# snimu/mixture-of-tokenizers

Hardware: AMD Instinct MI355X
Metric: mixed-embed tokens/sec at BxT=256x2048; achieved HBM GB/s vs peak (higher is better)
Workload: dtype f32

## Files before the change

### mixture-of-tokenizers_amd/csrc/mot_embed.hip

```cpp
#include <stdlib.h>

#include <algorithm>

#include "mot_wave.hpp"

namespace mot {

template <int MODE, int NCH, int U, typename T, bool DUAL>
struct MixStream {
    typedef typename Elem<T>::vec vec_t;
    typedef typename Elem<T>::raw raw_t;
    static constexpr int VEC = Elem<T>::kVec;
    const MixArgs &A;
    const WaveLds &W;
    const T *tok_table, *byte_table;
    int lane, Dm, nchunk, ntok;
    int tokv = 0, unit_lane0 = 0;
    bool act[NCH];
    bool tact[NCH];
    raw_t ar[U][NCH];

    __device__ __forceinline__ MixStream(const MixArgs &A_, const WaveLds &W_, int ntok_) : A(A_), W(W_), ntok(ntok_) {
        tok_table = (const T *)A.tok_table;
        byte_table = (const T *)A.byte_table;
        lane = threadIdx.x & 63;
        Dm = MODE == MOT_MIX_CONCAT ? A.Dt + A.bpt * A.Db : A.Dt;
        nchunk = Dm / VEC;
#pragma unroll
        for (int i = 0; i < NCH; ++i) act[i] = lane + 64 * i < nchunk;
        if (MODE == MOT_MIX_CONCAT) {
#pragma unroll
            for (int i = 0; i < NCH; ++i) tact[i] = VEC * (lane + 64 * i) < A.Dt;
        }
    }
    __device__ __forceinline__ void request(int tb) {
#pragma unroll
        for (int u = 0; u < U; ++u) {
            const int t = min(tb + u, ntok - 1);
            int tok = __builtin_amdgcn_readlane(tokv, unit_lane0 + t);
            if ((uint64_t)(uint32_t)tok >= (uint64_t)A.tok_rows) {
                if (A.status && lane == 0) atomicOr(A.status, kStatusTokenOor);
                tok = 0;
            }
            if (MODE == MOT_MIX_CONCAT) {
                const T *trow = tok_table + (int64_t)tok * A.Dt;
#pragma unroll
                for (int i = 0; i < NCH; ++i) ar[u][i] = Elem<T>::load_raw(trow + VEC * (tact[i] ? lane + 64 * i : 0));
                continue;
            }
            const T *trow = tok_table + (int64_t)tok * Dm;
#pragma unroll
            for (int i = 0; i < NCH; ++i) ar[u][i] = Elem<T>::load_raw(trow + VEC * (act[i] ? lane + 64 * i : 0));
        }
    }
    template <class RowOf>
    __device__ __forceinline__ void run(RowOf &&out_row) {
        constexpr bool dual = DUAL;
        const int sv = A.bpt | 1;
        int slot[NCH], within[NCH];
#pragma unroll
        for (int i = 0; i < NCH; ++i) {
            const int c = lane + 64 * i;
            const int cc = act[i] ? c : 0;
            if (MODE == MOT_MIX_SUM) {
                slot[i] = (VEC * cc) / A.Db;
                within[i] = VEC * cc - slot[i] * A.Db;
            } else if (MODE == MOT_MIX_CONCAT) {
                const int cb = (act[i] && !tact[i]) ? VEC * c - A.Dt : 0;
                slot[i] = cb / A.Db;
                within[i] = cb - slot[i] * A.Db;
            } else {
                slot[i] = 0;
                within[i] = VEC * cc;
            }
        }
        const float s_tok = A.scale_tok ? *A.scale_tok : 1.0f;
        const float s_byte = A.scale_byte ? *A.scale_byte : 1.0f;
        const bool scale_t = A.scale_tok != nullptr, scale_b = A.scale_byte != nullptr;
        auto sumsq = [](const vec_t &v) {
            float s = 0.f;
#pragma unroll
            for (int e = 0; e < VEC; ++e) s += v[e] * v[e];
            return s;
        };

        for (int tb = 0; tb < ntok; tb += U) {
            raw_t br[U][NCH], br2[DUAL ? U : 1][NCH];
            vec_t bm[U][NCH];
            int idr[U][NCH];
            if (tb > 0) request(tb);
#pragma unroll
            for (int u = 0; u < U; ++u) {
                const int t = min(tb + u, ntok - 1);
#pragma unroll
                for (int i = 0; i < NCH; ++i) {
                    if (MODE == MOT_MIX_SUM || MODE == MOT_MIX_CONCAT) {
                        const int id = W.ids[t * sv + slot[i]];
                        idr[u][i] = id;
                        br[u][i] = Elem<T>::load_raw(byte_table + (int64_t)id * A.Db + within[i]);
                        if (dual) br2[DUAL ? u : 0][i] = Elem<T>::load_raw(byte_table + (int64_t)W.ids2[t * sv + slot[i]] * A.Db + within[i]);
                    } else if (MODE == MOT_MIX_MEAN) {
                        vec_t acc = (vec_t)(0.f);
                        for (int k = 0; k < A.bpt; ++k) {
                            const int id = W.ids[t * sv + k];
                            vec_t v = Elem<T>::loadv(byte_table + (int64_t)id * A.Db + within[i]);
                            if (dual) {
                                const int id2 = W.ids2[t * sv + k];
                                v += Elem<T>::loadv(byte_table + (int64_t)id2 * A.Db + within[i]);
                            }
                            if (A.norm_byte) v *= A.byte_rnorm[id];
                            acc += v;
                        }
                        bm[u][i] = acc / (float)A.bpt;
                    }
                }
            }
#pragma unroll
            for (int u = 0; u < U; ++u) {
                const int t = tb + u;
                vec_t a[1][NCH], b[1][NCH];
#pragma unroll
                for (int i = 0; i < NCH; ++i) {
                    a[0][i] = Elem<T>::widen(ar[u][i]);
                    if (MODE == MOT_MIX_SUM) {
                        vec_t v = Elem<T>::widen(br[u][i]);
                        if (dual) v += Elem<T>::widen(br2[DUAL ? u : 0][i]);
                        if (A.norm_byte) v *= A.byte_rnorm[idr[u][i]];
                        b[0][i] = v;
                    } else if (MODE == MOT_MIX_CONCAT) {
                        vec_t v = Elem<T>::widen(br[u][i]);
                        if (dual) v += Elem<T>::widen(br2[DUAL ? u : 0][i]);
                        if (A.norm_byte) {
                            if (dual) {
                                float ss = sumsq(v);
                                for (int o = 1; o < A.Db / VEC; o <<= 1) ss += __shfl_xor(ss, o, 64);
                                v *= rms_scale(ss, A.Db, A.eps);
                            } else {
                                v *= A.byte_rnorm[idr[u][i]];
                            }
                        }
                        b[0][i] = v;
                    } else if (MODE == MOT_MIX_MEAN) {
                        b[0][i] = bm[u][i];
                    }
                }
                if (A.norm_tok) {
                    float ss = 0.f;
#pragma unroll
                    for (int i = 0; i < NCH; ++i) ss += (MODE == MOT_MIX_CONCAT ? tact[i] : act[i]) ? sumsq(a[0][i]) : 0.f;
                    const float r = rms_scale(wave_sum(ss), MODE == MOT_MIX_CONCAT ? A.Dt : Dm, A.eps);
#pragma unroll
                    for (int i = 0; i < NCH; ++i) a[0][i] *= r;
                }
                if (scale_t) {
#pragma unroll
                    for (int i = 0; i < NCH; ++i) a[0][i] *= s_tok;
                }
                vec_t x[NCH];
#pragma unroll
                for (int i = 0; i < NCH; ++i) {
                    if (MODE == MOT_MIX_NOOP) x[i] = a[0][i];
                    else if (MODE == MOT_MIX_CONCAT) x[i] = tact[i] ? a[0][i] : (scale_b ? b[0][i] * s_byte : b[0][i]);
                    else x[i] = a[0][i] + (scale_b ? b[0][i] * s_byte : b[0][i]);
                }
                if (A.norm_out) {
                    float ss = 0.f;
#pragma unroll
                    for (int i = 0; i < NCH; ++i) ss += act[i] ? sumsq(x[i]) : 0.f;
                    const float r = rms_scale(wave_sum(ss), Dm, A.eps);
#pragma unroll
                    for (int i = 0; i < NCH; ++i) x[i] *= r;
                }
                if (t < ntok) {
                    T *orow = out_row(t);
#pragma unroll
                    for (int i = 0; i < NCH; ++i)
                        if (act[i]) Elem<T>::storev_nt(orow + VEC * (lane + 64 * i), x[i]);
                }
            }
        }
    }
};

template <int MODE, int NCH, int U, typename T, bool DUAL>
__global__ __launch_bounds__(kThreads) void embed_mix_kernel(const MixArgs A) {
    extern __shared__ __attribute__((aligned(16))) unsigned char lds_wave[];
    constexpr bool has_ids = MODE != MOT_MIX_NOOP;
    constexpr bool dual = DUAL;
    const int lane = threadIdx.x & 63;
    const int wave = __builtin_amdgcn_readfirstlane(threadIdx.x >> 6);
    const int64_t unit_id = (int64_t)blockIdx.x * kWaves + wave;
    if (unit_id >= A.n_units) return;
    const int64_t row = unit_id / A.units_per_row;
    const int64_t u0 = (unit_id - row * A.units_per_row) * A.unit;
    const int ntok = (int)min((int64_t)A.unit, A.T - u0);
    const int stream_eb = (has_ids && A.id_source == MOT_IDS_FROM_TTB && A.pull_dir != kPullNone) ? A.ttb_elem : 0;
    const WaveLds W = wave_lds_carve(lds_wave + (size_t)wave * A.wave_lds, A.unit, has_ids ? A.bpt : 0, dual, stream_eb);
    MixStream<MODE, NCH, U, T, DUAL> S(A, W, ntok);

    auto from_ttb = [&](auto indexer) {
        S.tokv = indexer.tokens();
        S.unit_lane0 = indexer.unit_lane0;
        indexer.load_rows();
#ifndef MOT_VAR_NOPREFETCH
        S.request(0);
#endif
        indexer.finish();
#ifdef MOT_VAR_NOPREFETCH
        S.request(0);
#endif
    };
    if (has_ids && A.id_source == MOT_IDS_FROM_TTB) {
        if (A.ttb_elem == 2) {
            if (A.pull_dir == kPullLeft) from_ttb(WaveIndexer<kPullLeft, int16_t>(A, W, row, u0, ntok, dual));
            else if (A.pull_dir == kPullRight) from_ttb(WaveIndexer<kPullRight, int16_t>(A, W, row, u0, ntok, dual));
            else from_ttb(WaveIndexer<kPullNone, int16_t>(A, W, row, u0, ntok, dual));
        } else {
            if (A.pull_dir == kPullLeft) from_ttb(WaveIndexer<kPullLeft, int32_t>(A, W, row, u0, ntok, dual));
            else if (A.pull_dir == kPullRight) from_ttb(WaveIndexer<kPullRight, int32_t>(A, W, row, u0, ntok, dual));
            else from_ttb(WaveIndexer<kPullNone, int32_t>(A, W, row, u0, ntok, dual));
        }
    } else {
        S.tokv = lane < ntok ? A.tokens[row * A.T + u0 + lane] : 0;
        S.request(0);
        if (has_ids) wave_ids_given(A, W, row, u0, ntok);
        else if (A.counters && lane == 0) atomicAdd((unsigned long long *)A.counters, (unsigned long long)ntok);
    }

    T *orow = (T *)A.out + (row * A.T + u0) * (int64_t)S.Dm;
    S.run([&](int t) { return orow + (int64_t)t * S.Dm; });
}

constexpr int kRouteUnits = 8;
constexpr int64_t kRouteMinTokens = 131072;
constexpr int kClaimShards = 64;
constexpr int kClaimStride = 64;

struct RouteWs {
    uint32_t *claim;
    uint8_t *ends;
    uint8_t *offs;
    uint16_t *ids;
    uint16_t *ids2;
};

template <int DIR, typename E>
__global__ __launch_bounds__(kThreads) void route_index_kernel(const MixArgs A, const RouteWs R) {
    extern __shared__ __attribute__((aligned(16))) unsigned char lds_wave[];
    const int lane = threadIdx.x & 63;
    const int wave = __builtin_amdgcn_readfirstlane(threadIdx.x >> 6);
    if (blockIdx.x < 2) R.claim[(blockIdx.x * kThreads + threadIdx.x) * kClaimStride] = 0;
    const int64_t unit_id = (int64_t)blockIdx.x * kWaves + wave;
    if (unit_id >= A.n_units) return;
    const int64_t row = unit_id / A.units_per_row;
    const int64_t u0 = (unit_id - row * A.units_per_row) * A.unit;
    const int ntok = (int)min((int64_t)A.unit, A.T - u0);
    const bool dual = A.add_padded != 0;
    const WaveLds W = wave_lds_carve(lds_wave + (size_t)wave * A.wave_lds, A.unit, A.bpt, dual, DIR != kPullNone ? A.ttb_elem : 0);
    WaveIndexer<DIR, E> ix(A, W, row, u0, ntok, dual);
    const int tok = ix.tokens();
    ix.load_rows();
    ix.finish();

    const int bpt = A.bpt, sv = bpt | 1, n = ntok * bpt;
    const int64_t base = (row * A.T + u0) * bpt;
    for (int i = lane; i < n; i += 64) {
        const int t = i / bpt, k = i - t * bpt;
        R.ids[base + i] = (uint16_t)W.ids[t * sv + k];
        if (dual) R.ids2[base + i] = (uint16_t)W.ids2[t * sv + k];
    }
    const bool in = ix.in_unit;
    const int b = tok & 7;
    int rank = 0, end = 0, acc = 0;
#pragma unroll
    for (int q = 0; q < 8; ++q) {
        const unsigned long long m = __ballot(in && b == q);
        if (in && b == q) rank = acc + (int)__builtin_amdgcn_mbcnt_hi((unsigned)(m >> 32), __builtin_amdgcn_mbcnt_lo((unsigned)m, 0u));
        acc += __popcll(m);
        if (lane == q) end = acc;
    }
    if (in) R.offs[unit_id * A.unit + rank] = (uint8_t)ix.j;
    if (lane < 8) R.ends[unit_id * 8 + lane] = (uint8_t)end;
}

template <int NCH, int U, typename T, bool DUAL>
__global__ __launch_bounds__(kThreads) void embed_mix_routed_kernel(const MixArgs A, const RouteWs R) {
    extern __shared__ __attribute__((aligned(16))) unsigned char lds_wave[];
    const int lane = threadIdx.x & 63;
    const int wave = __builtin_amdgcn_readfirstlane(threadIdx.x >> 6);
    const WaveLds W = wave_lds_carve(lds_wave + (size_t)wave * A.wave_lds, 64, A.bpt, DUAL, 0);
    MixStream<MOT_MIX_SUM, NCH, U, T, DUAL> S(A, W, 0);
    const int bpt = A.bpt, sv = bpt | 1;
    const int64_t n_chunks = (A.n_units + kRouteUnits - 1) / kRouteUnits;
    const int home = blockIdx.x & 7;
    const int shard = ((blockIdx.x >> 3) * kWaves + wave) % kClaimShards;
    for (int q = 0; q < 8;) {
        const int b = (home + q) & 7;
        const int64_t lo = n_chunks * shard / kClaimShards, hi = n_chunks * (shard + 1) / kClaimShards;
        uint32_t k = 0;
        if (lane == 0) k = atomicAdd(R.claim + (b * kClaimShards + shard) * kClaimStride, 1u);
        const int64_t c = lo + __builtin_amdgcn_readfirstlane(k);
        if (c >= hi) { ++q; continue; }
        const int64_t uc = c * kRouteUnits;
        int nb = 0, sb = 0;
        if (lane < kRouteUnits && uc + lane < A.n_units) {
            const uint8_t *e = R.ends + (uc + lane) * 8;
            sb = b ? e[b - 1] : 0;
            nb = e[b] - sb;
        }
        const int incl = wave_scan_add(nb), excl = incl - nb;
        const int total = __builtin_amdgcn_readlane(incl, kRouteUnits - 1);
        for (int p0 = 0; p0 < total; p0 += 64) {
            const int l = p0 + lane;
            int g = 0;
#pragma unroll
            for (int gg = 1; gg < kRouteUnits; ++gg) g = l >= __builtin_amdgcn_readlane(excl, gg) ? gg : g;
            const int ex = __shfl(excl, g, 64), st = __shfl(sb, g, 64);
            int64_t pos = 0;
            int tok = 0;
            if (l < total) {
                const int64_t u = uc + g;
                const int64_t row = u / A.units_per_row;
                pos = row * A.T + (u - row * A.units_per_row) * A.unit + R.offs[u * A.unit + st + (l - ex)];
                tok = A.tokens[pos];
                if ((uint64_t)(uint32_t)tok >= (uint64_t)A.ttb_rows) tok = 0;
            }
            S.tokv = tok;
            S.ntok = min(64, total - p0);
            S.request(0);
            if (l < total) {
                const uint16_t *ia = R.ids + pos * bpt, *ib = R.ids2 + pos * bpt;
                if ((bpt & 7) == 0) {
                    typedef uint16_t u16x8 __attribute__((ext_vector_type(8)));
                    for (int k = 0; k < bpt; k += 8) {
                        const u16x8 va = *(const u16x8 *)(ia + k);
                        u16x8 vb;
                        if (DUAL) vb = *(const u16x8 *)(ib + k);
#pragma unroll
                        for (int e = 0; e < 8; ++e) {
                            W.ids[lane * sv + k + e] = va[e];
                            if (DUAL) W.ids2[lane * sv + k + e] = vb[e];
                        }
                    }
                } else {
                    for (int k = 0; k < bpt; ++k) {
                        W.ids[lane * sv + k] = ia[k];
                        if (DUAL) W.ids2[lane * sv + k] = ib[k];
                    }
                }
            }
            wave_lds_sync();
            const int plo = (int)(uint32_t)pos, phi = (int)(pos >> 32);
            S.run([&](int t) {
                const int64_t p = (int64_t)(((uint64_t)(uint32_t)__builtin_amdgcn_readlane(phi, t) << 32) |
                                            (uint32_t)__builtin_amdgcn_readlane(plo, t));
                return (T *)A.out + p * (int64_t)S.Dm;
            });
            wave_lds_sync();
        }
    }
}

template <typename T>
__global__ __launch_bounds__(kThreads) void rows_rnorm_kernel(const T *__restrict__ table, int64_t rows, int dim,
                                                              float eps, float *__restrict__ out) {
    const int lane = threadIdx.x & 63;
    const int64_t r = (int64_t)blockIdx.x * kWaves + (threadIdx.x >> 6);
    if (r >= rows) return;
    float ss = 0.f;
    for (int j = lane; j < dim; j += 64) {
        const float v = Elem<T>::load1(table + r * dim + j);
        ss += v * v;
    }
    ss = wave_sum(ss);
    if (lane == 0) out[r] = rms_scale(ss, dim, eps);
}

template <int G, typename IdT, typename T>
__global__ __launch_bounds__(kThreads) void gather_rows_kernel(const IdT *__restrict__ ids_a, const IdT *__restrict__ ids_b,
                                                               int64_t n, const T *__restrict__ table, int64_t rows,
                                                               int dim, int rms, float eps, const float *scale,
                                                               T *__restrict__ out, uint32_t *status, int group, int64_t out_ld,
                                                               uint32_t oor_flag) {
    const int g = threadIdx.x % G;
    const int64_t per_block = kThreads / G;
    const float s = scale ? *scale : 1.0f;
    const bool vec = (dim & 3) == 0;
    for (int64_t r = (int64_t)blockIdx.x * per_block + threadIdx.x / G; r < n; r += (int64_t)gridDim.x * per_block) {
        int64_t ia = (int64_t)ids_a[r], ib = ids_b ? (int64_t)ids_b[r] : 0;
        if ((uint64_t)ia >= (uint64_t)rows || (uint64_t)ib >= (uint64_t)rows) {
            if (status) atomicOr(status, oor_flag);
            if ((uint64_t)ia >= (uint64_t)rows) ia = 0;
            if ((uint64_t)ib >= (uint64_t)rows) ib = 0;
        }
        const T *pa = table + ia * dim, *pb = table + ib * dim;
        T *po = group == 1 ? out + r * out_ld : out + (r / group) * out_ld + (r % group) * dim;
        float mult = s;
        if (rms) {
            float ss = 0.f;
            if (vec) {
                for (int j = g; j < (dim >> 2); j += G) {
                    float4v v = Elem<T>::load4(pa + 4 * j);
                    if (ids_b) v += Elem<T>::load4(pb + 4 * j);
                    ss += v.x * v.x + v.y * v.y + v.z * v.z + v.w * v.w;
                }
            } else {
                for (int j = g; j < dim; j += G) {
                    float v = Elem<T>::load1(pa + j);
                    if (ids_b) v += Elem<T>::load1(pb + j);
                    ss += v * v;
                }
            }
#pragma unroll
            for (int o = G / 2; o > 0; o >>= 1) ss += __shfl_xor(ss, o, G);
            mult = rms_scale(ss, dim, eps);
        }
        if (vec) {
            for (int j = g; j < (dim >> 2); j += G) {
                float4v v = Elem<T>::load4(pa + 4 * j);
                if (ids_b) v += Elem<T>::load4(pb + 4 * j);
                if (rms) v *= mult;
                if (scale) v *= s;
                Elem<T>::store4_nt(po + 4 * j, v);
            }
        } else {
            for (int j = g; j < dim; j += G) {
                float v = Elem<T>::load1(pa + j);
                if (ids_b) v += Elem<T>::load1(pb + j);
                if (rms) v *= mult;
                if (scale) v *= s;
                Elem<T>::store1(po + j, v);
            }
        }
    }
}

template <int G, typename T>
static int launch_gather_g(const void *ids_a, const void *ids_b, int ids_elem, int64_t n, const void *table,
                           int64_t rows, int dim, int rms, float eps, const float *scale, void *out, uint32_t *status,
                           int group, int64_t out_ld, uint32_t oor_flag, hipStream_t stream) {
    const int64_t per_block = kThreads / G;
    int64_t blocks = (n + per_block - 1) / per_block;
    if (blocks > 256 * 128) blocks = 256 * 128;
    if (ids_elem == 8)
        hipLaunchKernelGGL((gather_rows_kernel<G, int64_t, T>), dim3((unsigned)blocks), dim3(kThreads), 0, stream,
                           (const int64_t *)ids_a, (const int64_t *)ids_b, n, (const T *)table, rows, dim, rms, eps, scale, (T *)out, status, group, out_ld, oor_flag);
    else
        hipLaunchKernelGGL((gather_rows_kernel<G, int32_t, T>), dim3((unsigned)blocks), dim3(kThreads), 0, stream,
                           (const int32_t *)ids_a, (const int32_t *)ids_b, n, (const T *)table, rows, dim, rms, eps, scale, (T *)out, status, group, out_ld, oor_flag);
    return check_launch("gather_rows_kernel");
}

template <typename T>
static int launch_gather_t(const void *ids_a, const void *ids_b, int ids_elem, int64_t n, const void *table, int64_t rows,
                           int dim, int rms_norm, float eps, const float *scale, void *out, uint32_t *status, int group, int64_t out_ld,
                           uint32_t oor_flag, hipStream_t stream) {
    const int lanes = (dim & 3) == 0 ? dim / 4 : dim;
    if (lanes <= 8) return launch_gather_g<8, T>(ids_a, ids_b, ids_elem, n, table, rows, dim, rms_norm, eps, scale, out, status, group, out_ld, oor_flag, stream);
    if (lanes <= 16) return launch_gather_g<16, T>(ids_a, ids_b, ids_elem, n, table, rows, dim, rms_norm, eps, scale, out, status, group, out_ld, oor_flag, stream);
    if (lanes <= 32) return launch_gather_g<32, T>(ids_a, ids_b, ids_elem, n, table, rows, dim, rms_norm, eps, scale, out, status, group, out_ld, oor_flag, stream);
    return launch_gather_g<64, T>(ids_a, ids_b, ids_elem, n, table, rows, dim, rms_norm, eps, scale, out, status, group, out_ld, oor_flag, stream);
}

int launch_gather_rows_placed(const void *ids_a, const void *ids_b, int ids_elem, int64_t n, const void *table, int64_t rows,
                              int dim, int rms_norm, float eps, const float *scale, void *out, int group, int64_t out_ld,
                              uint32_t *status, uint32_t oor_flag, int dtype, hipStream_t stream) {
    if (n == 0) return MOT_OK;
    if (eps <= 0.f) eps = dtype == MOT_BF16 ? 0.0078125f : FLT_EPSILON;
    if (dtype == MOT_BF16)
        return launch_gather_t<__bf16>(ids_a, ids_b, ids_elem, n, table, rows, dim, rms_norm, eps, scale, out, status, group, out_ld, oor_flag, stream);
    return launch_gather_t<float>(ids_a, ids_b, ids_elem, n, table, rows, dim, rms_norm, eps, scale, out, status, group, out_ld, oor_flag, stream);
}

int launch_gather_rows(const void *ids_a, const void *ids_b, int ids_elem, int64_t n, const void *table, int64_t rows,
                       int dim, int rms_norm, float eps, const float *scale, void *out, uint32_t *status, int dtype,
                       hipStream_t stream) {
    return launch_gather_rows_placed(ids_a, ids_b, ids_elem, n, table, rows, dim, rms_norm, eps, scale, out, 1, dim, status, kStatusByteOor, dtype,
                                     stream);
}

template <typename T>
__global__ __launch_bounds__(kThreads) void concat_rows_kernel(const int32_t *__restrict__ tokens, const int64_t *__restrict__ ids, int64_t n,
                                                               const T *__restrict__ tok_table, int64_t tok_rows, int Dt,
                                                               const T *__restrict__ byte_table, int64_t byte_rows, int Db, int bpt, int norm_tok,
                                                               const float *__restrict__ byte_rnorm, float eps, T *__restrict__ u, int K, int tok_lo,
                                                               int byte_lo, uint32_t *status) {
    using vec_t = typename Elem<T>::vec;
    constexpr int VEC = Elem<T>::kVec;
    const int lane = threadIdx.x & 63;
    const int64_t t = (int64_t)blockIdx.x * kWaves + (threadIdx.x >> 6);
    if (t >= n) return;
    int tok = tokens[t];
    if ((uint64_t)(uint32_t)tok >= (uint64_t)tok_rows) {
        if (status && lane == 0) atomicOr(status, kStatusTokenOor);
        tok = 0;
    }
    const T *trow = tok_table + (int64_t)tok * Dt;
    T *urow = u + t * K;
    const int nvt = Dt / VEC;
    float rs = 1.0f;
    if (norm_tok) {
        float ss = 0.f;
        for (int j = lane; j < nvt; j += 64) {
            const vec_t v = Elem<T>::loadv(trow + VEC * j);
#pragma unroll
            for (int e = 0; e < VEC; ++e) ss += v[e] * v[e];
        }
        rs = rms_scale(wave_sum(ss), Dt, eps);
    }
    for (int j = lane; j < nvt; j += 64) Elem<T>::storev_nt(urow + tok_lo + VEC * j, Elem<T>::loadv(trow + VEC * j) * rs);
    const int vps = Db / VEC, nvb = bpt * vps;
    for (int j = lane; j < nvb; j += 64) {
        const int slot = j / vps, within = (j - slot * vps) * VEC;
        int64_t id = ids[t * bpt + slot];
        if ((uint64_t)id >= (uint64_t)byte_rows) {
            if (status) atomicOr(status, kStatusByteOor);
            id = 0;
        }
        vec_t v = Elem<T>::loadv(byte_table + id * Db + within);
        if (byte_rnorm) v *= byte_rnorm[id];
        Elem<T>::storev_nt(urow + byte_lo + slot * Db + within, v);
    }
}

int launch_concat_rows(const int32_t *tokens, const int64_t *ids, int64_t n, const void *tok_table, int64_t tok_rows, int Dt, const void *byte_table,
                       int64_t byte_rows, int Db, int bpt, int norm_tok, const float *byte_rnorm, float eps, void *u, int K, int tok_lo, int byte_lo,
                       uint32_t *status, int dtype, hipStream_t stream) {
    if (n == 0) return MOT_OK;
    const unsigned blocks = (unsigned)((n + kWaves - 1) / kWaves);
    if (dtype == MOT_BF16)
        hipLaunchKernelGGL(concat_rows_kernel<__bf16>, dim3(blocks), dim3(kThreads), 0, stream, tokens, ids, n, (const __bf16 *)tok_table, tok_rows, Dt,
                           (const __bf16 *)byte_table, byte_rows, Db, bpt, norm_tok, byte_rnorm, eps, (__bf16 *)u, K, tok_lo, byte_lo, status);
    else
        hipLaunchKernelGGL(concat_rows_kernel<float>, dim3(blocks), dim3(kThreads), 0, stream, tokens, ids, n, (const float *)tok_table, tok_rows, Dt,
                           (const float *)byte_table, byte_rows, Db, bpt, norm_tok, byte_rnorm, eps, (float *)u, K, tok_lo, byte_lo, status);
    return check_launch("concat_rows_kernel");
}

int launch_rows_rnorm(const void *table, int64_t rows, int dim, float eps, float *out, int dtype, hipStream_t stream) {
    const int64_t rb = (rows + kWaves - 1) / kWaves;
    if (dtype == MOT_BF16)
        hipLaunchKernelGGL(rows_rnorm_kernel<__bf16>, dim3((unsigned)rb), dim3(kThreads), 0, stream, (const __bf16 *)table, rows, dim, eps, out);
    else
        hipLaunchKernelGGL(rows_rnorm_kernel<float>, dim3((unsigned)rb), dim3(kThreads), 0, stream, (const float *)table, rows, dim, eps, out);
    return check_launch("rows_rnorm_kernel");
}


static bool sum_routed(const MotEmbedMixDesc &d) {
    return d.mode == MOT_MIX_SUM && d.id_source == MOT_IDS_FROM_TTB && !d.out_ids_padded && !d.out_ids_pulled && d.bpt > 0 &&
           d.byte_rows <= 65536 && d.n_rows * d.tokens_per_row >= kRouteMinTokens && d.dtype == MOT_F32 &&
           (uint64_t)d.tok_rows * d.tok_dim * sizeof(float) <= ((uint64_t)256 << 20);
}

struct MixWorkspace {
    size_t rnorm, claim, ends, offs, ids, ids2, total;
};
static MixWorkspace mix_workspace(const MotEmbedMixDesc &d) {
    auto up = [](size_t x) { return (x + 255) & ~(size_t)255; };
    MixWorkspace w{};
    w.total = (d.mode != MOT_MIX_NOOP && d.norm_byte) ? up((size_t)d.byte_rows * sizeof(float)) : 0;
    if (!sum_routed(d)) return w;
    const int64_t tokens = d.n_rows * d.tokens_per_row;
    const int unit = pick_unit(tokens);
    const int64_t n_units = d.n_rows * ((d.tokens_per_row + unit - 1) / unit);
    const size_t id_bytes = up((size_t)tokens * d.bpt * sizeof(uint16_t));
    w.claim = w.total;
    w.ends = w.claim + (size_t)8 * kClaimShards * kClaimStride * sizeof(uint32_t);
    w.offs = w.ends + up((size_t)n_units * 8);
    w.ids = w.offs + up((size_t)n_units * unit);
    w.ids2 = w.ids + id_bytes;
    w.total = w.ids2 + (d.add_padded ? id_bytes : 0);
    return w;
}

size_t embed_mix_workspace_bytes(const MotEmbedMixDesc &d) {
    if (d.mode == MOT_MIX_CONCAT_LINEAR) return d.dtype == MOT_BF16 ? embed_mix_linear_bf16_workspace_bytes(d) : embed_mix_linear_workspace_bytes(d);
    return mix_workspace(d).total;
}

template <int DIR, typename E>
static void launch_route_index(const MixArgs &A, const RouteWs &R, int64_t blocks, size_t lds, hipStream_t stream) {
    hipLaunchKernelGGL((route_index_kernel<DIR, E>), dim3((unsigned)blocks), dim3(kThreads), lds, stream, A, R);
}

template <int NCH, int U, typename T, bool DUAL>
static int launch_routed(const MixArgs &A, const RouteWs &R, int64_t blocks, size_t lds, hipStream_t stream) {
    if (A.ttb_elem == 2) {
        if (A.pull_dir == kPullLeft) launch_route_index<kPullLeft, int16_t>(A, R, blocks, lds, stream);
        else if (A.pull_dir == kPullRight) launch_route_index<kPullRight, int16_t>(A, R, blocks, lds, stream);
        else launch_route_index<kPullNone, int16_t>(A, R, blocks, lds, stream);
    } else {
        if (A.pull_dir == kPullLeft) launch_route_index<kPullLeft, int32_t>(A, R, blocks, lds, stream);
        else if (A.pull_dir == kPullRight) launch_route_index<kPullRight, int32_t>(A, R, blocks, lds, stream);
        else launch_route_index<kPullNone, int32_t>(A, R, blocks, lds, stream);
    }
    if (int rc = check_launch("route_index_kernel")) return rc;
    MixArgs Ar = A;
    Ar.wave_lds = (int)wave_lds_bytes(64, A.bpt, DUAL, 0);
    const size_t lds_r = (size_t)Ar.wave_lds * kWaves;
    const void *kern = (const void *)embed_mix_routed_kernel<NCH, U, T, DUAL>;
    int dev = 0, cus = 0, per_cu = 0;
    if (hipGetDevice(&dev) != hipSuccess || hipDeviceGetAttribute(&cus, hipDeviceAttributeMultiprocessorCount, dev) != hipSuccess ||
        hipOccupancyMaxActiveBlocksPerMultiprocessor(&per_cu, kern, kThreads, lds_r) != hipSuccess || per_cu < 1)
        return set_error(MOT_EHIP, "embed_mix: no occupancy for embed_mix_routed_kernel");
    const int64_t grid = std::max<int64_t>(((int64_t)cus * per_cu) & ~(int64_t)7, 8 * kClaimShards / kWaves);
    hipLaunchKernelGGL((embed_mix_routed_kernel<NCH, U, T, DUAL>), dim3((unsigned)grid), dim3(kThreads), lds_r, stream, Ar, R);
    return check_launch("embed_mix_routed_kernel");
}

template <int MODE, int NCH, int U, typename T>
static int launch_mix(const MixArgs &A, int64_t blocks, size_t lds, hipStream_t stream, const RouteWs *route) {
    const bool dual = MODE != MOT_MIX_NOOP && (A.id_source == MOT_IDS_FROM_TTB ? A.add_padded != 0 : A.ids_b != nullptr);
    if constexpr (MODE == MOT_MIX_SUM && sizeof(T) == 4) {
        if (route) return dual ? launch_routed<NCH, U, T, true>(A, *route, blocks, lds, stream) : launch_routed<NCH, U, T, false>(A, *route, blocks, lds, stream);
    }
    if (dual)
        hipLaunchKernelGGL((embed_mix_kernel<MODE, NCH, U, T, true>), dim3((unsigned)blocks), dim3(kThreads), lds, stream, A);
    else
        hipLaunchKernelGGL((embed_mix_kernel<MODE, NCH, U, T, false>), dim3((unsigned)blocks), dim3(kThreads), lds, stream, A);
    return check_launch("embed_mix_kernel");
}

template <int MODE>
static int dispatch_nch(const MixArgs &A, int dtype, int64_t blocks, size_t lds, hipStream_t stream, const RouteWs *route = nullptr) {
    const int Dm = MODE == MOT_MIX_CONCAT ? A.Dt + A.bpt * A.Db : A.Dt;
    if (dtype == MOT_BF16) {
        switch ((Dm / 8 + 63) / 64) {
            case 1: return launch_mix<MODE, 1, 4, __bf16>(A, blocks, lds, stream, route);
            case 2: return launch_mix<MODE, 2, 4, __bf16>(A, blocks, lds, stream, route);
            case 3: return launch_mix<MODE, 3, 2, __bf16>(A, blocks, lds, stream, route);
            case 4: return launch_mix<MODE, 4, 2, __bf16>(A, blocks, lds, stream, route);
            default: return set_error(MOT_EUNSUPPORTED, "embed_mix: model_dim %d > 2048 is not built", Dm);
        }
    }
    switch ((Dm / 4 + 63) / 64) {
        case 1: return launch_mix<MODE, 1, 4, float>(A, blocks, lds, stream, route);
        case 2: return launch_mix<MODE, 2, 4, float>(A, blocks, lds, stream, route);
        case 3: return launch_mix<MODE, 3, 2, float>(A, blocks, lds, stream, route);
        case 4: return launch_mix<MODE, 4, 2, float>(A, blocks, lds, stream, route);
        case 5:
        case 6: return launch_mix<MODE, 6, 1, float>(A, blocks, lds, stream, route);
        case 7:
        case 8: return launch_mix<MODE, 8, 1, float>(A, blocks, lds, stream, route);
        default: return set_error(MOT_EUNSUPPORTED, "embed_mix: model_dim %d > 2048 is not built", Dm);
    }
}


template <typename T, int U, int BPT, bool NORMB, int ADD = 0>
__global__ __launch_bounds__(1024) void embed_mean_lds_kernel(const MixArgs A, int slice_cols, int nslices, int64_t tokens_per_part) {
    extern __shared__ __attribute__((aligned(16))) unsigned char lds_raw[];
    T *tab = (T *)lds_raw;
    constexpr int VEC = Elem<T>::kVec;
    typedef typename Elem<T>::vec vec_t;
    const int tid = threadIdx.x, lane = tid & 63, wave = tid >> 6;
    const int slice = blockIdx.x % nslices;
    const int64_t part = blockIdx.x / nslices;
    const int col0 = slice * slice_cols;
    const int D = A.Dt;
    const T *byte_table = (const T *)A.byte_table, *tok_table = (const T *)A.tok_table;
    const int pieces_per_row = slice_cols / VEC;
    for (int64_t q = tid; q < A.byte_rows * pieces_per_row; q += 1024) {
        const int r = (int)(q / pieces_per_row), c = (int)(q - (int64_t)r * pieces_per_row) * VEC;
        *(typename Elem<T>::raw *)(tab + (size_t)r * slice_cols + c) = Elem<T>::load_raw(byte_table + (int64_t)r * D + col0 + c);
    }
    __syncthreads();
    const float s_tok = A.scale_tok ? *A.scale_tok : 1.0f;
    const float s_byte = A.scale_byte ? *A.scale_byte : 1.0f;
    const float inv_bpt = 1.0f / (float)A.bpt;
    const int64_t n_all = A.T;
    const int64_t n0 = part * tokens_per_part, n1 = min(n_all, n0 + tokens_per_part);
    T *out = (T *)A.out;
    const int c = lane * VEC;
    const int64_t per_wave = (((n1 - n0 + 15) / 16) + U - 1) / U * U;
    const int64_t w_lo = min(n1, n0 + wave * per_wave), w_hi = min(n1, w_lo + per_wave);
    if (w_lo >= w_hi) return;
    const int id_lanes = U * A.bpt;
    int tokv_nx = w_lo + lane < w_hi ? A.tokens[w_lo + lane] : 0;
    for (int64_t chunk = w_lo; chunk < w_hi; chunk += 64) {
        const int tokv = tokv_nx;
        if (chunk + 64 < w_hi) tokv_nx = chunk + 64 + lane < w_hi ? A.tokens[chunk + 64 + lane] : 0;
        const int nb = (int)min((int64_t)64, w_hi - chunk);
        typename Elem<T>::raw ar_nx[U];
        uint2 old_nx[U];
        float4v old32_nx[U];
        int64_t id_nx = 0;
        auto request = [&](int b) {
#pragma unroll
            for (int u = 0; u < U; ++u) {
                int tok = __builtin_amdgcn_readlane(tokv, min(b + u, nb - 1));
                if ((uint64_t)(uint32_t)tok >= (uint64_t)A.tok_rows) {
                    if (A.status && lane == 0) atomicOr(A.status, kStatusTokenOor);
                    tok = 0;
                }
                ar_nx[u] = Elem<T>::load_raw(tok_table + (int64_t)tok * D + col0 + c);
                if constexpr (ADD == 1) old_nx[u] = *(const uint2 *)(A.add16 + (chunk + min(b + u, nb - 1)) * D + col0 + c);
                if constexpr (ADD == 2) old32_nx[u] = *(const float4v *)(A.out + (chunk + min(b + u, nb - 1)) * D + col0 + c);
            }
            const int64_t at = (chunk + b) * A.bpt + lane;
            id_nx = (lane < id_lanes && at < n_all * A.bpt) ? A.ids_a[at] : 0;
        };
        request(0);
        for (int b = 0; b < nb; b += U) {
            typename Elem<T>::raw ar[U];
            uint2 old[U];
            float4v old32[U];
#pragma unroll
            for (int u = 0; u < U; ++u) {
                ar[u] = ar_nx[u];
                if constexpr (ADD == 1) old[u] = old_nx[u];
                if constexpr (ADD == 2) old32[u] = old32_nx[u];
            }
            const int64_t idq = id_nx;
            if (b + U < nb) request(b + U);
            const bool bad = (uint64_t)idq >= (uint64_t)A.byte_rows;
            if (bad && A.status) atomicOr(A.status, kStatusByteOor);
            const int idv = bad ? 0 : (int)idq;
            const uint32_t row_bytes = (uint32_t)slice_cols * (uint32_t)sizeof(T);
            const uint32_t offv = (uint32_t)idv * row_bytes;
            const unsigned char *tabc = (const unsigned char *)tab + (size_t)c * sizeof(T);
            const int bpt = BPT ? BPT : A.bpt;
            const bool pow2 = (bpt & (bpt - 1)) == 0;
            const float cb = pow2 ? inv_bpt * s_byte : s_byte;
            T *orow = out + (chunk + b) * D + col0 + c;
#pragma unroll
            for (int u = 0; u < U; ++u) {
                vec_t acc0 = (vec_t)(0.f), acc1 = (vec_t)(0.f);
                const int l0 = u * bpt;
                auto one = [&](int k, vec_t &acc) {
                    const uint32_t so = (uint32_t)__builtin_amdgcn_readlane((int)offv, l0 + k);
                    vec_t v = Elem<T>::widen(*(const typename Elem<T>::raw *)(tabc + so));
                    if (NORMB) v *= A.byte_rnorm[__builtin_amdgcn_readlane(idv, l0 + k)];
                    acc += v;
                };
                if constexpr (BPT > 0) {
#pragma unroll
                    for (int k = 0; k < BPT; ++k) one(k, (k & 1) ? acc1 : acc0);
                } else {
                    int k = 0;
                    for (; k + 2 <= bpt; k += 2) { one(k, acc0); one(k + 1, acc1); }
                    if (k < bpt) one(k, acc0);
                }
                vec_t acc = acc0 + acc1;
                if (!pow2) acc = acc * inv_bpt;
                const vec_t x = Elem<T>::widen(ar[u]) * s_tok + acc * cb;
                if constexpr (ADD == 2) {
                    if (b + u < nb) Elem<float>::storev_nt((float *)orow + (int64_t)u * D, old32[u] + x);
                    continue;
                }
                if constexpr (ADD == 1) {
                    if (b + u < nb) {
                        const float4v h = {__uint_as_float(old[u].x << 16), __uint_as_float(old[u].x & 0xffff0000u), __uint_as_float(old[u].y << 16),
                                           __uint_as_float(old[u].y & 0xffff0000u)};
                        Elem<__bf16>::store4_nt(A.add16 + (chunk + b + u) * D + col0 + c, h + x);
                    }
                    continue;
                }
#ifdef MOT_C5_NOSTORE
                if (b + u < nb && x[0] == 123.456f)
#else
                if (b + u < nb)
#endif
                    Elem<T>::storev_nt(orow + (int64_t)u * D, x);
            }
        }
    }
}

template <typename T>
static int launch_mean_lds(MixArgs A, const MotEmbedMixDesc &d, int slice_cols, hipStream_t stream) {
    const int nslices = d.tok_dim / slice_cols;
    const int64_t N = d.n_rows * d.tokens_per_row;
    int64_t parts = 256 / nslices;
    if (parts < 1) parts = 1;
    const int64_t per = ((N + parts - 1) / parts + 63) & ~(int64_t)63;
    parts = (N + per - 1) / per;
    A.T = N;
    const size_t lds = (size_t)d.byte_rows * slice_cols * sizeof(T);
    static std::atomic<uint64_t> lds_ok{0};
    constexpr int kMeanU = 4;
#define MOT_MEAN_LAUNCH(BPT, NORMB)                                                                                                          \
    do {                                                                                                                                    \
        static std::atomic<uint64_t> ok_{0};                                                                           \
        if (int rc_lds = ensure_max_dyn_lds((const void *)embed_mean_lds_kernel<T, kMeanU, BPT, NORMB>, ok_, "embed_mean_lds_kernel")) return rc_lds; \
        hipLaunchKernelGGL((embed_mean_lds_kernel<T, kMeanU, BPT, NORMB>), dim3((unsigned)(parts * nslices)), dim3(1024), lds, stream, A, slice_cols, \
                           nslices, per);                                                                                                   \
    } while (0)
    (void)lds_ok;
    if constexpr (sizeof(T) == 4) {
        if (A.add16) {
            static std::atomic<uint64_t> ok_{0};
            if (d.norm_byte) return set_error(MOT_EUNSUPPORTED, "embed_mix: add16 without norm_byte");
            if (d.bpt == 8) {
                if (int rc_lds = ensure_max_dyn_lds((const void *)embed_mean_lds_kernel<T, kMeanU, 8, false, 1>, ok_, "embed_mean_lds_kernel")) return rc_lds;
                hipLaunchKernelGGL((embed_mean_lds_kernel<T, kMeanU, 8, false, 1>), dim3((unsigned)(parts * nslices)), dim3(1024), lds, stream, A, slice_cols, nslices, per);
            } else {
                static std::atomic<uint64_t> ok0_{0};
                if (int rc_lds = ensure_max_dyn_lds((const void *)embed_mean_lds_kernel<T, kMeanU, 0, false, 1>, ok0_, "embed_mean_lds_kernel")) return rc_lds;
                hipLaunchKernelGGL((embed_mean_lds_kernel<T, kMeanU, 0, false, 1>), dim3((unsigned)(parts * nslices)), dim3(1024), lds, stream, A, slice_cols, nslices, per);
            }
            return check_launch("embed_mean_lds_kernel");
        }
    }
    if constexpr (sizeof(T) == 4) {
        if (A.add_out) {
            if (d.norm_byte) return set_error(MOT_EUNSUPPORTED, "embed_mix: out += without norm_byte");
            if (d.bpt == 8) {
                static std::atomic<uint64_t> ok_{0};
                if (int rc_lds = ensure_max_dyn_lds((const void *)embed_mean_lds_kernel<T, kMeanU, 8, false, 2>, ok_, "embed_mean_lds_kernel")) return rc_lds;
                hipLaunchKernelGGL((embed_mean_lds_kernel<T, kMeanU, 8, false, 2>), dim3((unsigned)(parts * nslices)), dim3(1024), lds, stream, A, slice_cols, nslices, per);
            } else {
                static std::atomic<uint64_t> ok0_{0};
                if (int rc_lds = ensure_max_dyn_lds((const void *)embed_mean_lds_kernel<T, kMeanU, 0, false, 2>, ok0_, "embed_mean_lds_kernel")) return rc_lds;
                hipLaunchKernelGGL((embed_mean_lds_kernel<T, kMeanU, 0, false, 2>), dim3((unsigned)(parts * nslices)), dim3(1024), lds, stream, A, slice_cols, nslices, per);
            }
            return check_launch("embed_mean_lds_kernel");
        }
    }
    if (d.bpt == 8) { if (d.norm_byte) MOT_MEAN_LAUNCH(8, true); else MOT_MEAN_LAUNCH(8, false); }
    else { if (d.norm_byte) MOT_MEAN_LAUNCH(0, true); else MOT_MEAN_LAUNCH(0, false); }
#undef MOT_MEAN_LAUNCH
    return check_launch("embed_mean_lds_kernel");
}

static int mean_lds_slice(const MotEmbedMixDesc &d) {
    if (d.mode != MOT_MIX_MEAN || d.id_source != MOT_IDS_GIVEN || d.ids_b || d.norm_tok || d.norm_out || d.counters || d.out_ids_padded ||
        d.out_ids_pulled || (d.flags & MOT_FLAG_MEAN_GENERIC))
        return 0;
    const int esize = d.dtype == MOT_BF16 ? 2 : 4, chunk = 64 * (16 / esize);
    if (d.tok_dim % chunk || d.n_rows * d.tokens_per_row < 16384 || d.bpt * 4 > 64) return 0;
    const size_t budget = 144 * 1024;
    if ((size_t)d.byte_rows * chunk * esize > budget) return 0;
    return chunk;
}

bool embed_mix_mean_takes_add16(const MotEmbedMixDesc &d) { return d.dtype == MOT_F32 && mean_lds_slice(d) != 0; }

int launch_embed_mix(const MotEmbedMixDesc &d, hipStream_t stream, __bf16 *add16, bool add_out) {
    MixArgs A;
    fill_mix_args(A, d);
    A.add16 = add16;
    A.add_out = add_out ? 1 : 0;
    if ((add16 || add_out) && (d.dtype != MOT_F32 || !mean_lds_slice(d)))
        return set_error(MOT_EUNSUPPORTED, "embed_mix: add16 / out += are modes of the LDS-table MEAN kernel with fp32 tables");

    const bool has_ids = d.mode != MOT_MIX_NOOP;
    const bool dual = has_ids && (d.id_source == MOT_IDS_FROM_TTB ? d.add_padded != 0 : d.ids_b != nullptr);
    A.unit = pick_unit(d.n_rows * d.tokens_per_row);
#ifdef MOT_DEV_ABLATION
    if (getenv("MOT_UNIT") && atoi(getenv("MOT_UNIT")) > 0) A.unit = atoi(getenv("MOT_UNIT"));
#endif
    A.units_per_row = (d.tokens_per_row + A.unit - 1) / A.unit;
    A.n_units = d.n_rows * A.units_per_row;
    const int64_t blocks = (A.n_units + kWaves - 1) / kWaves;
    if (blocks > 0x7fffffffLL) return set_error(MOT_EUNSUPPORTED, "embed_mix: too many units");
    const int stream_eb = (has_ids && d.id_source == MOT_IDS_FROM_TTB && d.pull_dir != MOT_PULL_NONE) ? d.ttb_elem_bytes : 0;
    A.wave_lds = (int)wave_lds_bytes(A.unit, has_ids ? d.bpt : 0, dual, stream_eb);
    const size_t lds = (size_t)A.wave_lds * kWaves;

    const MixWorkspace ws = mix_workspace(d);
    if (ws.total && (!d.workspace || d.workspace_bytes < ws.total))
        return set_error(MOT_EWORKSPACE, "embed_mix: needs %zu workspace bytes, got %zu", ws.total, d.workspace_bytes);
    if (d.mode != MOT_MIX_NOOP && d.norm_byte) {
        float *rn = (float *)((unsigned char *)d.workspace + ws.rnorm);
        int rc = launch_rows_rnorm(d.byte_table, d.byte_rows, d.byte_dim, A.eps, rn, d.dtype, stream);
        if (rc) return rc;
        A.byte_rnorm = rn;
    }
    if (const int sc = mean_lds_slice(d)) {
        return d.dtype == MOT_BF16 ? launch_mean_lds<__bf16>(A, d, sc, stream) : launch_mean_lds<float>(A, d, sc, stream);
    }
    switch (d.mode) {
        case MOT_MIX_NOOP: return dispatch_nch<MOT_MIX_NOOP>(A, d.dtype, blocks, lds, stream);
        case MOT_MIX_SUM: {
            if (sum_routed(d) && A.unit == pick_unit(d.n_rows * d.tokens_per_row)) {
                unsigned char *w = (unsigned char *)d.workspace;
                const RouteWs R{(uint32_t *)(w + ws.claim), w + ws.ends, w + ws.offs, (uint16_t *)(w + ws.ids), (uint16_t *)(w + ws.ids2)};
                return dispatch_nch<MOT_MIX_SUM>(A, d.dtype, blocks, lds, stream, &R);
            }
            return dispatch_nch<MOT_MIX_SUM>(A, d.dtype, blocks, lds, stream);
        }
        case MOT_MIX_MEAN: return dispatch_nch<MOT_MIX_MEAN>(A, d.dtype, blocks, lds, stream);
        case MOT_MIX_CONCAT: return dispatch_nch<MOT_MIX_CONCAT>(A, d.dtype, blocks, lds, stream);
        default: return set_error(MOT_EINVAL, "embed_mix: bad mode %d", d.mode);
    }
}

}
```

### mixture-of-tokenizers_amd/csrc/mot_mix.hpp

```cpp
#pragma once
#include <float.h>

#include "mot_desc.hpp"
#include "mot_internal.hpp"
#include "mot_tile.hpp"

namespace mot {

typedef float float4v __attribute__((ext_vector_type(4)));
typedef float float8v __attribute__((ext_vector_type(8)));
typedef __bf16 bf16x4v __attribute__((ext_vector_type(4)));
typedef __bf16 bf16x8v __attribute__((ext_vector_type(8)));

template <typename T> struct Elem;
template <> struct Elem<float> {
    typedef float4v vec;
    typedef float4v raw;
    static constexpr int kVec = 4;
    static __device__ __forceinline__ raw load_raw(const float *p) { return *(const float4v *)p; }
    static __device__ __forceinline__ vec widen(raw r) { return r; }
    static __device__ __forceinline__ float4v loadv(const float *p) { return *(const float4v *)p; }
    static __device__ __forceinline__ void storev_nt(float *p, float4v v) { __builtin_nontemporal_store(v, (float4v *)p); }
    static __device__ __forceinline__ float4v load4(const float *p) { return *(const float4v *)p; }
    static __device__ __forceinline__ float load1(const float *p) { return *p; }
    static __device__ __forceinline__ void store4_nt(float *p, float4v v) { __builtin_nontemporal_store(v, (float4v *)p); }
    static __device__ __forceinline__ void store1(float *p, float v) { *p = v; }
};
template <> struct Elem<__bf16> {
    typedef float8v vec;
    typedef bf16x8v raw;
    static constexpr int kVec = 8;
    static __device__ __forceinline__ raw load_raw(const __bf16 *p) { return *(const bf16x8v *)p; }
    static __device__ __forceinline__ vec widen(raw r) { return __builtin_convertvector(r, float8v); }
    static __device__ __forceinline__ float8v loadv(const __bf16 *p) { return __builtin_convertvector(*(const bf16x8v *)p, float8v); }
    static __device__ __forceinline__ void storev_nt(__bf16 *p, float8v v) { __builtin_nontemporal_store(__builtin_convertvector(v, bf16x8v), (bf16x8v *)p); }
    static __device__ __forceinline__ float4v load4(const __bf16 *p) { return __builtin_convertvector(*(const bf16x4v *)p, float4v); }
    static __device__ __forceinline__ float load1(const __bf16 *p) { return (float)*p; }
    static __device__ __forceinline__ void store4_nt(__bf16 *p, float4v v) { __builtin_nontemporal_store(__builtin_convertvector(v, bf16x4v), (bf16x4v *)p); }
    static __device__ __forceinline__ void store1(__bf16 *p, float v) { *p = (__bf16)v; }
};

struct MixArgs {
    const int32_t *tokens;
    int64_t T;
    int bpt;
    int id_source, pull_dir;
    const void *ttb;
    int64_t ttb_rows;
    int ttb_elem;
    int add_padded;
    int32_t pad, eot;
    const int64_t *ids_a, *ids_b;
    const float *tok_table;
    int64_t tok_rows;
    int Dt;
    const float *byte_table;
    int64_t byte_rows;
    int Db;
    int norm_tok, norm_byte, norm_out;
    float eps;
    const float *scale_tok, *scale_byte;
    const float *byte_rnorm;
    float *out;
    __bf16 *add16;
    int add_out;
    int64_t *out_ids_padded, *out_ids_pulled, *counters;
    uint32_t *status;
    int tile_tokens, tiles_per_row;
    int unit, wave_lds;
    int64_t units_per_row, n_units;
};

constexpr float kBf16Eps = 0.0078125f;

__device__ __forceinline__ float rms_scale(float sumsq, int dim, float eps) {
    return __builtin_amdgcn_rsqf(sumsq * __builtin_amdgcn_rcpf((float)dim) + eps);
}

__device__ __forceinline__ int clamp_byte_id(int id, int64_t byte_rows, uint32_t *status) {
    if ((uint64_t)(uint32_t)id >= (uint64_t)byte_rows) {
        if (status) atomicOr(status, kStatusByteOor);
        return 0;
    }
    return id;
}

template <int DIR>
__device__ __forceinline__ void phase1_from_ttb(const MixArgs &A, const TileLds &L, int64_t row, int64_t t0, int ntok) {
    const int bpt = A.bpt, sv = bpt | 1;
    SrcTable src{A.tokens + row * A.T, A.ttb, A.ttb_rows, A.ttb_elem, bpt, A.pad, A.eot, A.status};
    if (DIR != kPullNone && (threadIdx.x >> 6) == kWaves - 1) halo_walk<DIR == kPullNone ? kPullLeft : DIR>(src, t0, ntok, A.T, bpt, L);
    fill_table_tile(src, t0, ntok, bpt, L);
    if (DIR != kPullNone) tile_scan_and_compact<DIR == kPullNone ? kPullLeft : DIR>(src, t0, ntok, A.T, bpt, L);
    const SlotLayout S(bpt);
    int pads_before = 0, pads_after = 0;
    if (S.kq < bpt) {
        const int64_t obase = (row * A.T + t0) * bpt;
        for (int t = S.tq; t < ntok; t += S.tstride) {
            const int own = L.val[t * sv + S.kq];
            int v = own;
            if (DIR != kPullNone) {
                int kind;
                const int payload = pulled_slot<DIR == kPullNone ? kPullLeft : DIR>(L, t, S.kq, ntok, bpt, &kind);
                v = kind == 1 ? A.pad : (kind == 2 ? own : payload);
            }
            if (A.out_ids_padded) A.out_ids_padded[obase + t * bpt + S.kq] = own;
            if (A.out_ids_pulled) A.out_ids_pulled[obase + t * bpt + S.kq] = v;
            pads_before += own == A.pad;
            pads_after += v == A.pad;
            L.ids[t * sv + S.kq] = clamp_byte_id(v, A.byte_rows, A.status);
        }
    }
    if (A.counters) {
        pads_before = (int)wave_sum((float)pads_before);
        pads_after = (int)wave_sum((float)pads_after);
        if ((threadIdx.x & 63) == 0) {
            atomicAdd((unsigned long long *)A.counters + 2, (unsigned long long)pads_before);
            atomicAdd((unsigned long long *)A.counters + 3, (unsigned long long)pads_after);
        }
        if (threadIdx.x == 0) {
            atomicAdd((unsigned long long *)A.counters + 0, (unsigned long long)ntok);
            atomicAdd((unsigned long long *)A.counters + 1, (unsigned long long)ntok * bpt);
        }
    }
    __syncthreads();
    if (A.add_padded && S.kq < bpt)
        for (int t = S.tq; t < ntok; t += S.tstride)
            L.val[t * sv + S.kq] = clamp_byte_id(L.val[t * sv + S.kq], A.byte_rows, A.status);
    __syncthreads();
}

__device__ __forceinline__ void phase1_given(const MixArgs &A, const TileLds &L, int64_t row, int64_t t0, int ntok) {
    const int bpt = A.bpt, sv = bpt | 1;
    if ((int)threadIdx.x < ntok) L.tok[threadIdx.x] = A.tokens[row * A.T + t0 + threadIdx.x];
    const SlotLayout S(bpt);
    if (S.kq < bpt) {
        const int64_t ibase = (row * A.T + t0) * bpt;
        for (int t = S.tq; t < ntok; t += S.tstride) {
            const int64_t a = A.ids_a[ibase + t * bpt + S.kq];
            int ia = (int)a;
            if ((uint64_t)a >= (uint64_t)A.byte_rows) { if (A.status) atomicOr(A.status, kStatusByteOor); ia = 0; }
            L.ids[t * sv + S.kq] = ia;
            if (A.ids_b) {
                const int64_t b = A.ids_b[ibase + t * bpt + S.kq];
                int ib = (int)b;
                if ((uint64_t)b >= (uint64_t)A.byte_rows) { if (A.status) atomicOr(A.status, kStatusByteOor); ib = 0; }
                L.val[t * sv + S.kq] = ib;
            }
        }
    }
    if (A.counters && threadIdx.x == 0) {
        atomicAdd((unsigned long long *)A.counters + 0, (unsigned long long)ntok);
        atomicAdd((unsigned long long *)A.counters + 1, (unsigned long long)ntok * bpt);
    }
    __syncthreads();
}


inline void fill_mix_ids(MixArgs &A, const IdSource &s) {
    A.tokens = s.tokens; A.T = s.tokens_per_row; A.bpt = s.bpt;
    A.id_source = s.id_source; A.pull_dir = s.pull_dir; A.ttb = s.ttb; A.ttb_rows = s.ttb_rows; A.ttb_elem = s.ttb_elem_bytes;
    A.add_padded = 0; A.pad = s.pad_byte; A.eot = s.eot_byte; A.ids_a = s.ids; A.ids_b = nullptr;
    A.out_ids_padded = s.out_ids_padded; A.out_ids_pulled = s.out_ids_pulled; A.counters = s.counters; A.status = s.status;
}

inline void fill_mix_args(MixArgs &A, const MotEmbedMixDesc &d) {
    fill_mix_ids(A, {d.tokens, d.n_rows, d.tokens_per_row, d.mode == MOT_MIX_NOOP ? 0 : d.bpt, d.id_source, d.pull_dir, d.ttb, d.ttb_rows,
                     d.ttb_elem_bytes, d.ids_a, d.pad_byte, d.eot_byte, d.out_ids_padded, d.out_ids_pulled, d.counters, d.status});
    A.add_padded = d.add_padded; A.ids_b = d.ids_b;
    A.tok_table = (const float *)d.tok_table; A.tok_rows = d.tok_rows; A.Dt = d.tok_dim;
    A.byte_table = (const float *)d.byte_table; A.byte_rows = d.byte_rows; A.Db = d.byte_dim;
    A.norm_tok = d.norm_tok; A.norm_byte = d.norm_byte; A.norm_out = d.norm_out;
    A.eps = d.eps > 0.f ? d.eps : (d.dtype == MOT_BF16 ? kBf16Eps : FLT_EPSILON);
    A.scale_tok = d.scale_tok; A.scale_byte = d.scale_byte;
    A.byte_rnorm = nullptr;
    A.out = (float *)d.out;
    A.add16 = nullptr;
    A.add_out = 0;
}

}
```

Measured before the change: 1.293 billion.

## Add compile-time route phases and buffer-store drop path to routed embed kernel

```diff
diff --git a/mixture-of-tokenizers_amd/csrc/mot_embed.hip b/mixture-of-tokenizers_amd/csrc/mot_embed.hip
--- a/mixture-of-tokenizers_amd/csrc/mot_embed.hip
+++ b/mixture-of-tokenizers_amd/csrc/mot_embed.hip
@@ -6,7 +6,7 @@
 
 namespace mot {
 
-template <int MODE, int NCH, int U, typename T, bool DUAL>
+template <int MODE, int NCH, int U, typename T, bool DUAL, bool DROP = false>
 struct MixStream {
     typedef typename Elem<T>::vec vec_t;
     typedef typename Elem<T>::raw raw_t;
@@ -173,9 +173,16 @@
                 }
                 if (t < ntok) {
                     T *orow = out_row(t);
-#pragma unroll
-                    for (int i = 0; i < NCH; ++i)
-                        if (act[i]) Elem<T>::storev_nt(orow + VEC * (lane + 64 * i), x[i]);
+                    if (DROP) {
+                        const __amdgpu_buffer_rsrc_t rs = drop_row(orow, Dm * (int)sizeof(T));
+#pragma unroll
+                        for (int i = 0; i < NCH; ++i)
+                            if (act[i]) Elem<T>::storev_drop(rs, VEC * lane, VEC * 64 * i, x[i]);
+                    } else {
+#pragma unroll
+                        for (int i = 0; i < NCH; ++i)
+                            if (act[i]) Elem<T>::storev_nt(orow + VEC * (lane + 64 * i), x[i]);
+                    }
                 }
             }
         }
@@ -231,7 +238,20 @@
     S.run([&](int t) { return orow + (int64_t)t * S.Dm; });
 }
 
-constexpr int kRouteUnits = 8;
+#ifdef MOT_VAR_ROUTE_PHASES
+constexpr int kRoutePhases = MOT_VAR_ROUTE_PHASES;
+#else
+constexpr int kRoutePhases = 1;
+#endif
+#ifdef MOT_VAR_ROUTE_DROP
+constexpr bool kRouteDrop = true;
+#else
+constexpr bool kRouteDrop = false;
+#endif
+constexpr int kRouteKeys = 8 * kRoutePhases;
+constexpr int kRouteUnits = kRouteKeys;
+static_assert(kRoutePhases >= 1 && (kRoutePhases & (kRoutePhases - 1)) == 0 && kRouteKeys <= 64, "one key and one unit of a chunk per lane");
+__device__ __forceinline__ int route_key(int tok) { return (tok & 7) * kRoutePhases + ((tok >> 3) & (kRoutePhases - 1)); }
 constexpr int64_t kRouteMinTokens = 131072;
 constexpr int kClaimShards = 64;
 constexpr int kClaimStride = 64;
@@ -270,17 +290,18 @@
         if (dual) R.ids2[base + i] = (uint16_t)W.ids2[t * sv + k];
     }
     const bool in = ix.in_unit;
-    const int b = tok & 7;
-    int rank = 0, end = 0, acc = 0;
-#pragma unroll
-    for (int q = 0; q < 8; ++q) {
-        const unsigned long long m = __ballot(in && b == q);
-        if (in && b == q) rank = acc + (int)__builtin_amdgcn_mbcnt_hi((unsigned)(m >> 32), __builtin_amdgcn_mbcnt_lo((unsigned)m, 0u));
-        acc += __popcll(m);
-        if (lane == q) end = acc;
-    }
+    const int key = route_key(tok);
+    unsigned long long same = __ballot(in), same_k = same;
+    int less = 0, less_k = 0;
+#pragma unroll
+    for (int bit = kRouteKeys >> 1; bit >= 1; bit >>= 1) {
+        const unsigned long long m = __ballot(in && (key & bit));
+        if (key & bit) { less += __popcll(same & ~m); same &= m; } else same &= ~m;
+        if (lane & bit) { less_k += __popcll(same_k & ~m); same_k &= m; } else same_k &= ~m;
+    }
+    const int rank = less + (int)__builtin_amdgcn_mbcnt_hi((unsigned)(same >> 32), __builtin_amdgcn_mbcnt_lo((unsigned)same, 0u));
     if (in) R.offs[unit_id * A.unit + rank] = (uint8_t)ix.j;
-    if (lane < 8) R.ends[unit_id * 8 + lane] = (uint8_t)end;
+    if (lane < kRouteKeys) R.ends[unit_id * kRouteKeys + lane] = (uint8_t)(less_k + __popcll(same_k));
 }
 
 template <int NCH, int U, typename T, bool DUAL>
@@ -289,24 +310,28 @@
     const int lane = threadIdx.x & 63;
     const int wave = __builtin_amdgcn_readfirstlane(threadIdx.x >> 6);
     const WaveLds W = wave_lds_carve(lds_wave + (size_t)wave * A.wave_lds, 64, A.bpt, DUAL, 0);
-    MixStream<MOT_MIX_SUM, NCH, U, T, DUAL> S(A, W, 0);
+    MixStream<MOT_MIX_SUM, NCH, U, T, DUAL, kRouteDrop> S(A, W, 0);
     const int bpt = A.bpt, sv = bpt | 1;
     const int64_t n_chunks = (A.n_units + kRouteUnits - 1) / kRouteUnits;
     const int home = blockIdx.x & 7;
     const int shard = ((blockIdx.x >> 3) * kWaves + wave) % kClaimShards;
+    const int64_t lo = n_chunks * shard / kClaimShards, hi = n_chunks * (shard + 1) / kClaimShards;
+    const uint32_t nc = (uint32_t)(hi - lo);
     for (int q = 0; q < 8;) {
         const int b = (home + q) & 7;
-        const int64_t lo = n_chunks * shard / kClaimShards, hi = n_chunks * (shard + 1) / kClaimShards;
         uint32_t k = 0;
         if (lane == 0) k = atomicAdd(R.claim + (b * kClaimShards + shard) * kClaimStride, 1u);
-        const int64_t c = lo + __builtin_amdgcn_readfirstlane(k);
-        if (c >= hi) { ++q; continue; }
+        k = __builtin_amdgcn_readfirstlane(k);
+        if (k >= nc * kRoutePhases) { ++q; continue; }
+        const uint32_t phase = k / nc;
+        const int64_t c = lo + (k - phase * nc);
         const int64_t uc = c * kRouteUnits;
+        const int key = b * kRoutePhases + (int)phase;
         int nb = 0, sb = 0;
         if (lane < kRouteUnits && uc + lane < A.n_units) {
-            const uint8_t *e = R.ends + (uc + lane) * 8;
-            sb = b ? e[b - 1] : 0;
-            nb = e[b] - sb;
+            const uint8_t *e = R.ends + (uc + lane) * kRouteKeys;
+            sb = key ? e[key - 1] : 0;
+            nb = e[key] - sb;
         }
         const int incl = wave_scan_add(nb), excl = incl - nb;
         const int total = __builtin_amdgcn_readlane(incl, kRouteUnits - 1);
@@ -314,7 +339,7 @@
             const int l = p0 + lane;
             int g = 0;
 #pragma unroll
-            for (int gg = 1; gg < kRouteUnits; ++gg) g = l >= __builtin_amdgcn_readlane(excl, gg) ? gg : g;
+            for (int s = kRouteUnits >> 1; s >= 1; s >>= 1) g = __shfl(excl, g + s, 64) <= l ? g + s : g;
             const int ex = __shfl(excl, g, 64), st = __shfl(sb, g, 64);
             int64_t pos = 0;
             int tok = 0;
@@ -567,7 +592,7 @@
     const size_t id_bytes = up((size_t)tokens * d.bpt * sizeof(uint16_t));
     w.claim = w.total;
     w.ends = w.claim + (size_t)8 * kClaimShards * kClaimStride * sizeof(uint32_t);
-    w.offs = w.ends + up((size_t)n_units * 8);
+    w.offs = w.ends + up((size_t)n_units * kRouteKeys);
     w.ids = w.offs + up((size_t)n_units * unit);
     w.ids2 = w.ids + id_bytes;
     w.total = w.ids2 + (d.add_padded ? id_bytes : 0);
diff --git a/mixture-of-tokenizers_amd/csrc/mot_mix.hpp b/mixture-of-tokenizers_amd/csrc/mot_mix.hpp
--- a/mixture-of-tokenizers_amd/csrc/mot_mix.hpp
+++ b/mixture-of-tokenizers_amd/csrc/mot_mix.hpp
@@ -11,6 +11,12 @@
 typedef float float8v __attribute__((ext_vector_type(8)));
 typedef __bf16 bf16x4v __attribute__((ext_vector_type(4)));
 typedef __bf16 bf16x8v __attribute__((ext_vector_type(8)));
+typedef unsigned int uint4v __attribute__((ext_vector_type(4)));
+
+__device__ __forceinline__ __amdgpu_buffer_rsrc_t drop_row(void *row, int bytes) {
+    return __builtin_amdgcn_make_buffer_rsrc(row,  0, bytes, 0x00020000);
+}
+constexpr int kAuxSc1 = 16;
 
 template <typename T> struct Elem;
 template <> struct Elem<float> {
@@ -21,6 +27,9 @@
     static __device__ __forceinline__ vec widen(raw r) { return r; }
     static __device__ __forceinline__ float4v loadv(const float *p) { return *(const float4v *)p; }
     static __device__ __forceinline__ void storev_nt(float *p, float4v v) { __builtin_nontemporal_store(v, (float4v *)p); }
+    static __device__ __forceinline__ void storev_drop(__amdgpu_buffer_rsrc_t row, int lane_col, int wave_col, float4v v) {
+        __builtin_amdgcn_raw_buffer_store_b128(__builtin_bit_cast(uint4v, v), row, lane_col * 4, wave_col * 4, kAuxSc1);
+    }
     static __device__ __forceinline__ float4v load4(const float *p) { return *(const float4v *)p; }
     static __device__ __forceinline__ float load1(const float *p) { return *p; }
     static __device__ __forceinline__ void store4_nt(float *p, float4v v) { __builtin_nontemporal_store(v, (float4v *)p); }
@@ -34,6 +43,9 @@
     static __device__ __forceinline__ vec widen(raw r) { return __builtin_convertvector(r, float8v); }
     static __device__ __forceinline__ float8v loadv(const __bf16 *p) { return __builtin_convertvector(*(const bf16x8v *)p, float8v); }
     static __device__ __forceinline__ void storev_nt(__bf16 *p, float8v v) { __builtin_nontemporal_store(__builtin_convertvector(v, bf16x8v), (bf16x8v *)p); }
+    static __device__ __forceinline__ void storev_drop(__amdgpu_buffer_rsrc_t row, int lane_col, int wave_col, float8v v) {
+        __builtin_amdgcn_raw_buffer_store_b128(__builtin_bit_cast(uint4v, __builtin_convertvector(v, bf16x8v)), row, lane_col * 2, wave_col * 2, kAuxSc1);
+    }
     static __device__ __forceinline__ float4v load4(const __bf16 *p) { return __builtin_convertvector(*(const bf16x4v *)p, float4v); }
     static __device__ __forceinline__ float load1(const __bf16 *p) { return (float)*p; }
     static __device__ __forceinline__ void store4_nt(__bf16 *p, float4v v) { __builtin_nontemporal_store(__builtin_convertvector(v, bf16x4v), (bf16x4v *)p); }
```

After: 1.293 billion, median of 2. Within noise of the previous version (+0.0%).
